# lms-org/trajectory_controller

Hardware: AMD Instinct MI355X
Metric: MPC QP solves/sec (horizon N=20, 2 inputs) at 1/2/4/8 MI355X; max|du| vs dlib (higher is better)
Workload: dtype f64; 1 GPU; batch 262144 trajectories per GPU, N=20, 2 inputs, compact (mpcControllerTobi) form, cold start, eps 0.01, max_iter 10000; global_batch=262144, horizon=20, algo=lane_fma, parallelism=batch-sharded x1, batches_in_flight=1, gather=none (1 GPU)

## Files before the change

trajectory_controller_amd/csrc/mpc_ub.h:

```cpp
#pragma once

#include "mpc_lane.h"
#include "mpc_ub_model.h"

namespace tpc {

template <typename T, bool EQB> TPC_DEV void ub_set_uniform(ub::Unit<T, EQB>& m, T gscale, const CompactArgs& g) {
    const T q[2] = {(T)g.q[0], (T)g.q[1]}, r[2] = {(T)g.r[0], (T)g.r[1]};
    const T lo[2] = {(T)g.lo[0], (T)g.lo[1]}, hi[2] = {(T)g.hi[0], (T)g.hi[1]};
    m.set_uniform(gscale, q, r, lo, hi);
}

template <typename T, int H> struct UbCdPlan {
    static constexpr bool mirror = 2 * (2 * H * kWave * (int)sizeof(T)) <= 64 * 1024 &&
                                   2 * (2 * H * kWave * (int)sizeof(T)) * 4 * CdOcc<T, H>::value <= 160 * 1024;
    static constexpr bool x_in_lds = mirror && sizeof(T) == 8 && H >= 20;
    static constexpr bool fast = true;
};

TPC_DEV double cd_ldexp(double x, int e) { return __builtin_ldexp(x, e); }
TPC_DEV float cd_ldexp(float x, int e) { return __builtin_ldexpf(x, e); }

template <typename T, int H, bool EQB>
__global__ __launch_bounds__(64, (CdOcc<T, H>::value)) void ub_cd_kernel(CompactArgs g, Knobs kn, T* __restrict__ recs,
                                                                         uint32_t* __restrict__ keys,
                                                                         uint32_t* __restrict__ key_rank,
                                                                         uint32_t* __restrict__ key_hist,
                                                                         unsigned long long* __restrict__ stats) {
    using P = UbCdPlan<T, H>;
    constexpr int RL = LaneRec<T, H>::kLen;
    constexpr bool MIRROR = P::mirror, XL = P::x_in_lds;
    __shared__ T s_iqd[2 * H][kWave];
    __shared__ T s_x[MIRROR ? 2 * H : 1][kWave];
    const int lane = threadIdx.x;
    const int64_t k = (int64_t)blockIdx.x * kWave + lane;
    if (k >= g.n) return;

    ub::Unit<T, EQB> m;
    ub_set_uniform(m, (T)1, g);
    const T ty = ((const T*)g.dy)[k], tphi = ((const T*)g.dphi)[k];
    m.set_instance((T)g.step, (T)g.wheelbase, ((const T*)g.v)[k], ty, tphi);
    const bool nonfinite = m.nonfinite_inputs(ty, tphi);
    const T q0 = (T)g.q[0], q1 = (T)g.q[1], r0 = (T)g.r[0], r1 = (T)g.r[1];

    T x[XL ? 1 : 2 * H], w[ub::Reverse<T, H>::value ? 1 : 2 * H];
    auto X = [&](int q) -> T { if constexpr (XL) return s_x[q][lane]; else return x[q]; };
#pragma unroll
    for (int q = 0; q < 2 * H; ++q) {
        if constexpr (!XL) x[q] = m.xz(q & 1);
        if constexpr (MIRROR) s_x[q][lane] = m.xz(q & 1);
    }
    const T lambda = ub::ctor_lambda_qdiag<T, H>(m.a, m.c, q0, q1, r0, r1, [&](int i, int j, T val) {
        s_iqd[2 * i + j][lane] = val != (T)0 ? (T)1 / (val * m.s(j)) : (T)0;
    });
    const T eps = (T)kn.eps;
    const bool screen_ok = ub::fast_stop_ok(m, ty, tphi, q0, q1, r0, r1, eps, lambda);
    const unsigned long long failing = __ballot(!screen_ok);
    if (failing != 0ull && lane == __ffsll((long long)failing) - 1) atomicOr(&stats[2], 1ull);
    if constexpr (sizeof(T) == 4) {
        const unsigned long long unmoved = __ballot(!ub::moved_stop_ok(m, eps, lambda));
        if (unmoved != 0ull && lane == __ffsll((long long)unmoved) - 1) atomicOr(&stats[2], 2ull);
    }
    const uint32_t cd_iters = kn.smo_iters < kn.max_iter ? kn.smo_iters : kn.max_iter;
    uint32_t iter = 0;
    bool stopped = nonfinite;
    bool vinit = false;
    constexpr T kHuge = (T)(sizeof(T) == 8 ? 0x1p600 : 0x1p100);
    T huge = kHuge;
    asm volatile("" : "+v"(huge));

    auto iteration = [&](auto fast_tag, uint32_t it) {
        constexpr bool F = decltype(fast_tag)::value;
        constexpr bool RV = ub::Reverse<T, H>::value;
        T Z, Y;
        m.fwd_init(Z, Y);
#pragma unroll
        for (int i = 0; i < H; ++i) {
            m.fwd(Z, Y, X(2 * i), X(2 * i + 1));
            if constexpr (!RV) { w[2 * i] = Z; w[2 * i + 1] = Y; }
        }
        T n0, n1;
        m.bwd_last(n0, n1, Z, Y);
        T max_df = (T)0, best_x = (T)0, best_mm = (T)0;
        int best = 0, best_sign = 0;
#pragma unroll
        for (int i = H - 1; i >= 0; --i) {
            if (i < H - 1) {
                if constexpr (RV) m.bwd(n0, n1, Z, Y); else m.bwd(n0, n1, w[2 * i], w[2 * i + 1]);
            }
            const T xi[2] = {X(2 * i), X(2 * i + 1)};
#pragma unroll
            for (int j = 1; j >= 0; --j) {
                const int q = 2 * i + j;
                const T xx = xi[j];
                const T dd = j == 0 ? m.df0(n1, xx) : m.df1(n0, n1, xx);
                if constexpr (F) {
                    T g_lo, g_hi;
                    if constexpr (ub::Unit<T, EQB>::kUnitBox) { g_lo = cd_ldexp(xx, 1900); g_hi = cd_ldexp((T)1 - xx, 1900); }
                    else { g_lo = m.gap_lo(j, xx, huge); g_hi = m.gap_hi(j, xx, huge); }
                    const T mm = tmax(tmin(dd, g_lo), -g_hi);
                    const bool better = tabs(mm) >= tabs(best_mm);
                    best_mm = better ? mm : best_mm;
                    best = better ? q : best;
                    if constexpr (!MIRROR) best_x = better ? xx : best_x;
                } else {
                    const T up = (xx <= m.bl(j)) ? (T)0 : dd;
                    const T dn = (xx >= m.bh(j)) ? (T)0 : -dd;
                    const T mag = tmax(up, dn);
                    const bool better = mag >= max_df && mag > (T)0;
                    max_df = tmax(max_df, mag);
                    best = better ? q : best;
                    best_sign = better ? sign_word(dd) : best_sign;
                    if constexpr (!MIRROR) best_x = better ? xx : best_x;
                }
            }
            if constexpr (RV) { if (i > 0) m.rev(Z, Y, xi[0], xi[1]); }
        }
        if constexpr (F) max_df = tabs(best_mm);
        stopped = stopped || max_df < eps;
        const bool act = !stopped;
        T best_df;
        if constexpr (F) best_df = best_mm; else best_df = with_sign(max_df, best_sign);
        if constexpr (MIRROR) best_x = s_x[best][lane];
        const T iq = s_iqd[best][lane];
        const bool upd = act && iq != (T)0;
        const T nx = m.project(ub::fma_(-iq, best_df, best_x), best & 1);
        if constexpr (MIRROR) { if (upd) s_x[best][lane] = nx; }
        if constexpr (!XL) {
            const int sel = upd ? best : -1;
#pragma unroll
            for (int q = 0; q < 2 * H; ++q) x[q] = (q == sel) ? nx : x[q];
        }
        vinit = upd ? (it + 1 == kn.smo_iters) : vinit;
        iter += act ? 1u : 0u;
    };
    if (P::fast && failing == 0ull) {
#pragma unroll 1
        for (uint32_t it = 0; it < cd_iters; ++it) {
            if (__ballot(!stopped) == 0ull) break;
            iteration(std::true_type{}, it);
        }
    } else {
#pragma unroll 1
        for (uint32_t it = 0; it < cd_iters; ++it) {
            if (__ballot(!stopped) == 0ull) break;
            iteration(std::false_type{}, it);
        }
    }

    T* rec = recs + (int64_t)k * RL;
#pragma unroll
    for (int q = 0; q < 2 * H; ++q) rec[q] = X(q);
    rec[2 * H] = lambda;
    uint64_t meta = (uint64_t)iter;
    if (stopped) meta |= kMetaStopped;
    if (vinit) meta |= kMetaVInit;
    if (nonfinite) meta |= kMetaNonFinite;
    store_meta<T>(rec + 2 * H + 1, meta);
    {
        T il0, il1, beta;
        ub::pg_constants<T>(lambda, m.s0, m.s1, il0, il1, beta);
        T* ex = rec + LaneRec<T, H>::kExtra;
        ex[0] = il0; ex[1] = il1; ex[2] = beta; ex[3] = m.a; ex[4] = m.c; ex[5] = ty; ex[6] = tphi;
    }
    const bool finished = stopped || iter >= kn.max_iter;
    const T lambda_floor = (r0 + r1) * (T)H;
    const bool uninformative = lambda < (T)1.5 * lambda_floor;
    const float lf = g.work_hint ? (float)(g.work_hint[k] > 0 ? g.work_hint[k] : 1) : (float)lambda;
    const uint32_t spread = (uint32_t)k & 127u;
    uint32_t key = __float_as_uint(lf);
    if (finished) key = spread << 16;
    else if (!g.work_hint && uninformative) key = (0x7f00u + spread) << 16;
    else if (!(lf > 0.0f) || key < 0x00800000u) key = 0x00800000u;
    else if (key >= 0x7f000000u) key = 0x7effffffu;
    uint32_t f = 0;
    if (finished) {
        ((T*)g.front)[k] = nonfinite ? (T)0 : m.control(0, X(0));
        ((T*)g.rear)[k] = nonfinite ? (T)0 : m.control(1, X(1));
        if (g.iters) g.iters[k] = (int32_t)iter;
        if (nonfinite) f |= 0x1u;
        if (!stopped) f |= 0x2u;
    }
    raise_flags(g.flags, f);
    keys[k] = key;
    key_rank[k] = atomicAdd(&key_hist[key >> 16], 1u);
}

#ifndef TPC_UB_OCC
#define TPC_UB_OCC 0
#endif
#ifndef TPC_UB_KV
#define TPC_UB_KV -1
#endif
template <typename T, int H> struct UbPlan {
    static constexpr bool D = sizeof(T) == 8;
    static constexpr int words = D ? 2 : 1;
    static constexpr bool reverse = ub::Reverse<T, H>::value;
    static constexpr bool regs = 6 * H * words <= 200 || !D || (reverse && 4 * H * words <= 200);
    static constexpr int occ_default = D ? 1 : ((H == 10 || H == 20) ? 2 : 1);
    static constexpr int occ = TPC_UB_OCC > 0 ? TPC_UB_OCC : occ_default;
    static constexpr int kv_default = regs ? H : (H == 20 ? 16 : (H == 30 ? 8 : 16));
    static constexpr int kv = regs ? H : (TPC_UB_KV >= 0 ? TPC_UB_KV : kv_default);
    static constexpr bool step_barrier = H - kv >= 8;
};
template <int H> struct UbRefillBatch { static constexpr int value = RefillBatch<H>::value; };

template <typename T, int H, bool EQB, int MODE>
__global__ __launch_bounds__((64 * UbPlan<T, H>::occ), (UbPlan<T, H>::occ)) void ub_pg_kernel(
    CompactArgs g, Knobs kn, const T* __restrict__ recs, const uint32_t* __restrict__ order,
    uint32_t* __restrict__ ticket, unsigned long long* __restrict__ stats, const uint32_t* __restrict__ queue_len) {
    using P = UbPlan<T, H>;
    constexpr int RL = LaneRec<T, H>::kLen;
    const int64_t n_queue = (int64_t)__builtin_nontemporal_load(queue_len);
    constexpr bool FAST = MODE != 0;
    static_assert(MODE == 0 || MODE == 2 || (MODE == 1 && sizeof(T) == 4), "the mask-as-arithmetic build is fp32's");
    {
        const unsigned long long sel = __builtin_nontemporal_load(&stats[2]);
        const int need = (sel & 1ull) ? 0 : ((sizeof(T) == 4 && (sel & 2ull)) ? 1 : 2);
        if (need != MODE) return;
        if (n_queue <= 0) return;
    }
    constexpr int BT = kWave * P::occ;
    constexpr int KV = P::kv, VL = H - KV;
// ... 213 lines not shown
```

Before: 58.23 million solves/s.

## Replace f64 coordinate-descent inner loop with hand-scheduled inline GCN assembly

For f64, H=20 with equality bounds and x in LDS, the fast coordinate-descent loop is replaced by a generated inline-asm loop. It batches LDS reads with explicit waitcnt interleaving, runs the forward and backward recurrences as FMA chains, does the argmax selection with cndmask, and writes the projected update back to LDS under an exec mask. The two shared arrays are merged into one contiguous buffer so fixed st64 offsets can address them. This is meant to cut compiler scheduling overhead and per-iteration branching. In exchange it hard-codes about 178 VGPRs, which may limit occupancy. It also uses a clamp-based projection and ldexp bounds tricks that must match the C++ semantics.

```diff
diff --git a/trajectory_controller_amd/csrc/mpc_ub.h b/trajectory_controller_amd/csrc/mpc_ub.h
--- a/trajectory_controller_amd/csrc/mpc_ub.h
+++ b/trajectory_controller_amd/csrc/mpc_ub.h
@@ -2,6 +2,7 @@
 
 #include "mpc_lane.h"
 #include "mpc_ub_model.h"
+#include "mpc_ub_cd_asm.h"
 
 namespace tpc {
 
@@ -16,6 +17,14 @@
                                    2 * (2 * H * kWave * (int)sizeof(T)) * 4 * CdOcc<T, H>::value <= 160 * 1024;
     static constexpr bool x_in_lds = mirror && sizeof(T) == 8 && H >= 20;
     static constexpr bool fast = true;
+};
+
+template <typename T, int H, bool EQB> struct UbCdAsm {
+#ifdef TPC_UB_CD_NO_ASM
+    static constexpr bool value = false;
+#else
+    static constexpr bool value = sizeof(T) == 8 && H == kUbCdAsmH && EQB && UbCdPlan<T, H>::x_in_lds;
+#endif
 };
 
 TPC_DEV double cd_ldexp(double x, int e) { return __builtin_ldexp(x, e); }
@@ -30,8 +39,9 @@
     using P = UbCdPlan<T, H>;
     constexpr int RL = LaneRec<T, H>::kLen;
     constexpr bool MIRROR = P::mirror, XL = P::x_in_lds;
-    __shared__ T s_iqd[2 * H][kWave];
-    __shared__ T s_x[MIRROR ? 2 * H : 1][kWave];
+    __shared__ T s_cd[2 * H + (MIRROR ? 2 * H : 1)][kWave];
+    T (*const s_iqd)[kWave] = s_cd;
+    T (*const s_x)[kWave] = s_cd + 2 * H;
     const int lane = threadIdx.x;
     const int64_t k = (int64_t)blockIdx.x * kWave + lane;
     if (k >= g.n) return;
@@ -135,10 +145,21 @@
         iter += act ? 1u : 0u;
     };
     if (P::fast && failing == 0ull) {
+        if constexpr (UbCdAsm<T, H, EQB>::value) {
+            static_assert(kUbCdAsmXRow == 2 * H, "LDS layout the generated loop reads");
+            const UbCdAsmUniform u = {m.gq0, m.gq1, m.grs0, m.grs1, m.lo1, (double)kn.eps};
+            uint64_t live = __ballot(!stopped);
+            uint32_t lu = 0;
+            const uint32_t vaddr = (uint32_t)(uintptr_t)&s_cd[0][lane];
+            ub_cd_asm_loop(u, m.a, m.c, m.as1, m.cs0, m.z0, m.q1th, m.grl0, m.grl1, vaddr, cd_iters, live, iter, lu);
+            stopped = ((live >> lane) & 1ull) == 0ull;
+            vinit = lu != 0u && lu == kn.smo_iters;
+        } else {
 #pragma unroll 1
-        for (uint32_t it = 0; it < cd_iters; ++it) {
-            if (__ballot(!stopped) == 0ull) break;
-            iteration(std::true_type{}, it);
+            for (uint32_t it = 0; it < cd_iters; ++it) {
+                if (__ballot(!stopped) == 0ull) break;
+                iteration(std::true_type{}, it);
+            }
         }
     } else {
 #pragma unroll 1
diff --git a/trajectory_controller_amd/csrc/mpc_ub_cd_asm.h b/trajectory_controller_amd/csrc/mpc_ub_cd_asm.h
--- /dev/null
+++ b/trajectory_controller_amd/csrc/mpc_ub_cd_asm.h
@@ -0,0 +1,667 @@
+#pragma once
+
+namespace tpc {
+
+constexpr int kUbCdAsmH = 20, kUbCdAsmIterInstrs = 627, kUbCdAsmXRow = 40;
+
+struct UbCdAsmUniform { double gq0, gq1, grs0, grs1, lo1, eps; };
+#pragma clang diagnostic push
+#pragma clang diagnostic ignored "-Winline-asm"
+TPC_DEV void ub_cd_asm_loop(const UbCdAsmUniform& u, double a, double c, double as1, double cs0, double z0, double q1th,
+                            double grl0, double grl1, uint32_t vaddr, uint32_t cd_iters, uint64_t& live,
+                            uint32_t& iter, uint32_t& lu) {
+    uint64_t sexec;
+    uint32_t sit;
+    asm volatile(
+        "s_waitcnt lgkmcnt(0)\n"
+        "s_mov_b64 %[sexec], exec\n"
+        "s_mov_b32 %[sit], 0\n"
+        ".p2align 3\n"
+        "TOP%=:\n"
+        "s_cmp_ge_u32 %[sit], %[scd]\n"
+        "s_cbranch_scc1 END%=\n"
+        "s_cmp_eq_u64 %[slive], 0\n"
+        "s_cbranch_scc1 END%=\n"
+        "ds_read2st64_b64 v[0:3], %[vaddr] offset0:40 offset1:41\n"
+        "ds_read2st64_b64 v[4:7], %[vaddr] offset0:42 offset1:43\n"
+        "ds_read2st64_b64 v[8:11], %[vaddr] offset0:44 offset1:45\n"
+        "ds_read2st64_b64 v[12:15], %[vaddr] offset0:46 offset1:47\n"
+        "ds_read2st64_b64 v[16:19], %[vaddr] offset0:48 offset1:49\n"
+        "ds_read2st64_b64 v[20:23], %[vaddr] offset0:50 offset1:51\n"
+        "ds_read2st64_b64 v[24:27], %[vaddr] offset0:52 offset1:53\n"
+        "ds_read2st64_b64 v[28:31], %[vaddr] offset0:54 offset1:55\n"
+        "ds_read2st64_b64 v[32:35], %[vaddr] offset0:56 offset1:57\n"
+        "ds_read2st64_b64 v[36:39], %[vaddr] offset0:58 offset1:59\n"
+        "ds_read2st64_b64 v[40:43], %[vaddr] offset0:60 offset1:61\n"
+        "ds_read2st64_b64 v[44:47], %[vaddr] offset0:62 offset1:63\n"
+        "ds_read2st64_b64 v[48:51], %[vaddr] offset0:64 offset1:65\n"
+        "ds_read2st64_b64 v[52:55], %[vaddr] offset0:66 offset1:67\n"
+        "ds_read2st64_b64 v[56:59], %[vaddr] offset0:68 offset1:69\n"
+        "s_waitcnt lgkmcnt(13)\n"
+        "s_nop 0\n"
+        "v_fma_f64 v[80:81], %[ca], %[slo1], %[cz0]\n"
+        "v_fma_f64 v[82:83], -%[ccs], v[2:3], %[slo1]\n"
+        "v_fma_f64 v[80:81], %[cas], v[2:3], v[80:81]\n"
+        "v_fma_f64 v[82:83], %[ccs], v[0:1], v[82:83]\n"
+        "ds_read2st64_b64 v[60:63], %[vaddr] offset0:70 offset1:71\n"
+        "v_fma_f64 v[84:85], %[ca], v[82:83], v[80:81]\n"
+        "v_fma_f64 v[86:87], -%[ccs], v[6:7], v[82:83]\n"
+        "v_fma_f64 v[84:85], %[cas], v[6:7], v[84:85]\n"
+        "v_fma_f64 v[86:87], %[ccs], v[4:5], v[86:87]\n"
+        "ds_read2st64_b64 v[64:67], %[vaddr] offset0:72 offset1:73\n"
+        "s_waitcnt lgkmcnt(13)\n"
+        "s_nop 0\n"
+        "v_fma_f64 v[88:89], %[ca], v[86:87], v[84:85]\n"
+        "v_fma_f64 v[90:91], -%[ccs], v[10:11], v[86:87]\n"
+        "v_fma_f64 v[88:89], %[cas], v[10:11], v[88:89]\n"
+        "v_fma_f64 v[90:91], %[ccs], v[8:9], v[90:91]\n"
+        "ds_read2st64_b64 v[68:71], %[vaddr] offset0:74 offset1:75\n"
+        "v_fma_f64 v[92:93], %[ca], v[90:91], v[88:89]\n"
+        "v_fma_f64 v[94:95], -%[ccs], v[14:15], v[90:91]\n"
+        "v_fma_f64 v[92:93], %[cas], v[14:15], v[92:93]\n"
+        "v_fma_f64 v[94:95], %[ccs], v[12:13], v[94:95]\n"
+        "ds_read2st64_b64 v[72:75], %[vaddr] offset0:76 offset1:77\n"
+        "s_waitcnt lgkmcnt(11)\n"
+        "s_nop 0\n"
+        "v_fma_f64 v[96:97], %[ca], v[94:95], v[92:93]\n"
+        "v_fma_f64 v[98:99], -%[ccs], v[18:19], v[94:95]\n"
+        "v_fma_f64 v[96:97], %[cas], v[18:19], v[96:97]\n"
+        "v_fma_f64 v[98:99], %[ccs], v[16:17], v[98:99]\n"
+        "ds_read2st64_b64 v[76:79], %[vaddr] offset0:78 offset1:79\n"
+        "v_fma_f64 v[100:101], %[ca], v[98:99], v[96:97]\n"
+        "v_fma_f64 v[102:103], -%[ccs], v[22:23], v[98:99]\n"
+        "v_fma_f64 v[100:101], %[cas], v[22:23], v[100:101]\n"
+        "v_fma_f64 v[102:103], %[ccs], v[20:21], v[102:103]\n"
+        "v_fma_f64 v[104:105], %[ca], v[102:103], v[100:101]\n"
+        "v_fma_f64 v[106:107], -%[ccs], v[26:27], v[102:103]\n"
+        "v_fma_f64 v[104:105], %[cas], v[26:27], v[104:105]\n"
+        "v_fma_f64 v[106:107], %[ccs], v[24:25], v[106:107]\n"
+        "v_fma_f64 v[108:109], %[ca], v[106:107], v[104:105]\n"
+        "v_fma_f64 v[110:111], -%[ccs], v[30:31], v[106:107]\n"
+        "v_fma_f64 v[108:109], %[cas], v[30:31], v[108:109]\n"
+        "v_fma_f64 v[110:111], %[ccs], v[28:29], v[110:111]\n"
+        "s_waitcnt lgkmcnt(8)\n"
+        "s_nop 0\n"
+        "v_fma_f64 v[112:113], %[ca], v[110:111], v[108:109]\n"
+        "v_fma_f64 v[114:115], -%[ccs], v[34:35], v[110:111]\n"
+        "v_fma_f64 v[112:113], %[cas], v[34:35], v[112:113]\n"
+        "v_fma_f64 v[114:115], %[ccs], v[32:33], v[114:115]\n"
+        "v_fma_f64 v[116:117], %[ca], v[114:115], v[112:113]\n"
+        "v_fma_f64 v[118:119], -%[ccs], v[38:39], v[114:115]\n"
+        "v_fma_f64 v[116:117], %[cas], v[38:39], v[116:117]\n"
+        "v_fma_f64 v[118:119], %[ccs], v[36:37], v[118:119]\n"
+        "v_fma_f64 v[120:121], %[ca], v[118:119], v[116:117]\n"
+        "v_fma_f64 v[122:123], -%[ccs], v[42:43], v[118:119]\n"
+        "v_fma_f64 v[120:121], %[cas], v[42:43], v[120:121]\n"
+        "v_fma_f64 v[122:123], %[ccs], v[40:41], v[122:123]\n"
+        "v_fma_f64 v[124:125], %[ca], v[122:123], v[120:121]\n"
+        "v_fma_f64 v[126:127], -%[ccs], v[46:47], v[122:123]\n"
+        "v_fma_f64 v[124:125], %[cas], v[46:47], v[124:125]\n"
+        "v_fma_f64 v[126:127], %[ccs], v[44:45], v[126:127]\n"
+        "s_waitcnt lgkmcnt(4)\n"
+        "s_nop 0\n"
+        "v_fma_f64 v[128:129], %[ca], v[126:127], v[124:125]\n"
+        "v_fma_f64 v[130:131], -%[ccs], v[50:51], v[126:127]\n"
+        "v_fma_f64 v[128:129], %[cas], v[50:51], v[128:129]\n"
+        "v_fma_f64 v[130:131], %[ccs], v[48:49], v[130:131]\n"
+        "v_fma_f64 v[132:133], %[ca], v[130:131], v[128:129]\n"
+        "v_fma_f64 v[134:135], -%[ccs], v[54:55], v[130:131]\n"
+        "v_fma_f64 v[132:133], %[cas], v[54:55], v[132:133]\n"
+        "v_fma_f64 v[134:135], %[ccs], v[52:53], v[134:135]\n"
+        "v_fma_f64 v[136:137], %[ca], v[134:135], v[132:133]\n"
+        "v_fma_f64 v[138:139], -%[ccs], v[58:59], v[134:135]\n"
+        "v_fma_f64 v[136:137], %[cas], v[58:59], v[136:137]\n"
+        "v_fma_f64 v[138:139], %[ccs], v[56:57], v[138:139]\n"
+        "v_fma_f64 v[140:141], %[ca], v[138:139], v[136:137]\n"
+        "v_fma_f64 v[142:143], -%[ccs], v[62:63], v[138:139]\n"
+        "v_fma_f64 v[140:141], %[cas], v[62:63], v[140:141]\n"
+        "v_fma_f64 v[142:143], %[ccs], v[60:61], v[142:143]\n"
+        "s_waitcnt lgkmcnt(0)\n"
+        "s_nop 0\n"
+        "v_fma_f64 v[144:145], %[ca], v[142:143], v[140:141]\n"
+        "v_fma_f64 v[146:147], -%[ccs], v[66:67], v[142:143]\n"
+        "v_fma_f64 v[144:145], %[cas], v[66:67], v[144:145]\n"
+        "v_fma_f64 v[146:147], %[ccs], v[64:65], v[146:147]\n"
+        "v_fma_f64 v[148:149], %[ca], v[146:147], v[144:145]\n"
+        "v_fma_f64 v[150:151], -%[ccs], v[70:71], v[146:147]\n"
+        "v_fma_f64 v[148:149], %[cas], v[70:71], v[148:149]\n"
+        "v_fma_f64 v[150:151], %[ccs], v[68:69], v[150:151]\n"
+        "v_fma_f64 v[152:153], %[ca], v[150:151], v[148:149]\n"
+        "v_fma_f64 v[154:155], -%[ccs], v[74:75], v[150:151]\n"
+        "v_fma_f64 v[152:153], %[cas], v[74:75], v[152:153]\n"
+        "v_fma_f64 v[154:155], %[ccs], v[72:73], v[154:155]\n"
+        "v_fma_f64 v[156:157], %[ca], v[154:155], v[152:153]\n"
+        "v_fma_f64 v[158:159], -%[ccs], v[78:79], v[154:155]\n"
+        "v_fma_f64 v[156:157], %[cas], v[78:79], v[156:157]\n"
+        "v_fma_f64 v[158:159], %[ccs], v[76:77], v[158:159]\n"
+        "v_mul_f64 v[160:161], %[sgq0], v[156:157]\n"
+        "v_fma_f64 v[162:163], %[sgq1], v[158:159], -%[cq]\n"
+        "v_fma_f64 v[164:165], %[sgrs1], v[78:79], %[cgl1]\n"
+        "v_fma_f64 v[164:165], -%[cc], v[162:163], v[164:165]\n"
+        "v_fma_f64 v[164:165], %[ca], v[160:161], v[164:165]\n"
+        "v_ldexp_f64 v[166:167], v[78:79], %[s1900]\n"
+        "v_fma_f64 v[168:169], -v[78:79], %[sbig], %[sbig]\n"
+        "v_min_f64 v[170:171], v[164:165], v[166:167]\n"
+        "v_max_f64 v[170:171], v[170:171], -v[168:169]\n"
+        "v_fma_f64 v[164:165], %[sgrs0], v[76:77], %[cgl0]\n"
+        "v_fma_f64 v[164:165], %[cc], v[162:163], v[164:165]\n"
+        "v_ldexp_f64 v[166:167], v[76:77], %[s1900]\n"
+        "v_fma_f64 v[168:169], -v[76:77], %[sbig], %[sbig]\n"
+        "v_min_f64 v[166:167], v[164:165], v[166:167]\n"
+        "v_max_f64 v[166:167], v[166:167], -v[168:169]\n"
+        "v_cmp_lt_f64_e64 vcc, |v[166:167]|, |v[170:171]|\n"
+        "v_cndmask_b32_e64 v170, v166, v170, vcc\n"
+        "v_cndmask_b32_e64 v171, v167, v171, vcc\n"
+        "v_cndmask_b32_e64 v172, 38, 39, vcc\n"
+        "v_fma_f64 v[154:155], %[sgq1], v[154:155], -%[cq]\n"
+        "v_fma_f64 v[162:163], %[ca], v[160:161], v[162:163]\n"
+        "v_add_f64 v[162:163], v[162:163], v[154:155]\n"
+        "v_fma_f64 v[160:161], %[sgq0], v[152:153], v[160:161]\n"
+        "v_fma_f64 v[164:165], %[sgrs1], v[74:75], %[cgl1]\n"
+        "v_fma_f64 v[164:165], -%[cc], v[162:163], v[164:165]\n"
+        "v_fma_f64 v[164:165], %[ca], v[160:161], v[164:165]\n"
+        "v_ldexp_f64 v[166:167], v[74:75], %[s1900]\n"
+        "v_fma_f64 v[168:169], -v[74:75], %[sbig], %[sbig]\n"
+        "v_min_f64 v[166:167], v[164:165], v[166:167]\n"
+        "v_max_f64 v[166:167], v[166:167], -v[168:169]\n"
+        "v_cmp_lt_f64_e64 vcc, |v[166:167]|, |v[170:171]|\n"
+        "v_cndmask_b32_e64 v170, v166, v170, vcc\n"
+        "v_cndmask_b32_e64 v171, v167, v171, vcc\n"
+        "v_cndmask_b32_e64 v172, 37, v172, vcc\n"
+        "v_fma_f64 v[164:165], %[sgrs0], v[72:73], %[cgl0]\n"
+        "v_fma_f64 v[164:165], %[cc], v[162:163], v[164:165]\n"
+        "v_ldexp_f64 v[166:167], v[72:73], %[s1900]\n"
+        "v_fma_f64 v[168:169], -v[72:73], %[sbig], %[sbig]\n"
+        "v_min_f64 v[166:167], v[164:165], v[166:167]\n"
+        "v_max_f64 v[166:167], v[166:167], -v[168:169]\n"
+        "v_cmp_lt_f64_e64 vcc, |v[166:167]|, |v[170:171]|\n"
+        "v_cndmask_b32_e64 v170, v166, v170, vcc\n"
+        "v_cndmask_b32_e64 v171, v167, v171, vcc\n"
+        "v_cndmask_b32_e64 v172, 36, v172, vcc\n"
+        "v_fma_f64 v[150:151], %[sgq1], v[150:151], -%[cq]\n"
+        "v_fma_f64 v[162:163], %[ca], v[160:161], v[162:163]\n"
+        "v_add_f64 v[162:163], v[162:163], v[150:151]\n"
+        "v_fma_f64 v[160:161], %[sgq0], v[148:149], v[160:161]\n"
+        "v_fma_f64 v[164:165], %[sgrs1], v[70:71], %[cgl1]\n"
+        "v_fma_f64 v[164:165], -%[cc], v[162:163], v[164:165]\n"
+        "v_fma_f64 v[164:165], %[ca], v[160:161], v[164:165]\n"
+        "v_ldexp_f64 v[166:167], v[70:71], %[s1900]\n"
+        "v_fma_f64 v[168:169], -v[70:71], %[sbig], %[sbig]\n"
+        "v_min_f64 v[166:167], v[164:165], v[166:167]\n"
+        "v_max_f64 v[166:167], v[166:167], -v[168:169]\n"
+        "v_cmp_lt_f64_e64 vcc, |v[166:167]|, |v[170:171]|\n"
+        "v_cndmask_b32_e64 v170, v166, v170, vcc\n"
+        "v_cndmask_b32_e64 v171, v167, v171, vcc\n"
+        "v_cndmask_b32_e64 v172, 35, v172, vcc\n"
+        "v_fma_f64 v[164:165], %[sgrs0], v[68:69], %[cgl0]\n"
+        "v_fma_f64 v[164:165], %[cc], v[162:163], v[164:165]\n"
+        "v_ldexp_f64 v[166:167], v[68:69], %[s1900]\n"
+        "v_fma_f64 v[168:169], -v[68:69], %[sbig], %[sbig]\n"
+        "v_min_f64 v[166:167], v[164:165], v[166:167]\n"
+        "v_max_f64 v[166:167], v[166:167], -v[168:169]\n"
+        "v_cmp_lt_f64_e64 vcc, |v[166:167]|, |v[170:171]|\n"
+        "v_cndmask_b32_e64 v170, v166, v170, vcc\n"
+        "v_cndmask_b32_e64 v171, v167, v171, vcc\n"
+        "v_cndmask_b32_e64 v172, 34, v172, vcc\n"
+        "v_fma_f64 v[146:147], %[sgq1], v[146:147], -%[cq]\n"
+        "v_fma_f64 v[162:163], %[ca], v[160:161], v[162:163]\n"
+        "v_add_f64 v[162:163], v[162:163], v[146:147]\n"
+        "v_fma_f64 v[160:161], %[sgq0], v[144:145], v[160:161]\n"
+        "v_fma_f64 v[164:165], %[sgrs1], v[66:67], %[cgl1]\n"
+        "v_fma_f64 v[164:165], -%[cc], v[162:163], v[164:165]\n"
+        "v_fma_f64 v[164:165], %[ca], v[160:161], v[164:165]\n"
+        "v_ldexp_f64 v[166:167], v[66:67], %[s1900]\n"
+        "v_fma_f64 v[168:169], -v[66:67], %[sbig], %[sbig]\n"
+        "v_min_f64 v[166:167], v[164:165], v[166:167]\n"
+        "v_max_f64 v[166:167], v[166:167], -v[168:169]\n"
+        "v_cmp_lt_f64_e64 vcc, |v[166:167]|, |v[170:171]|\n"
+        "v_cndmask_b32_e64 v170, v166, v170, vcc\n"
+        "v_cndmask_b32_e64 v171, v167, v171, vcc\n"
+        "v_cndmask_b32_e64 v172, 33, v172, vcc\n"
+        "v_fma_f64 v[164:165], %[sgrs0], v[64:65], %[cgl0]\n"
+        "v_fma_f64 v[164:165], %[cc], v[162:163], v[164:165]\n"
+        "v_ldexp_f64 v[166:167], v[64:65], %[s1900]\n"
+        "v_fma_f64 v[168:169], -v[64:65], %[sbig], %[sbig]\n"
+        "v_min_f64 v[166:167], v[164:165], v[166:167]\n"
+        "v_max_f64 v[166:167], v[166:167], -v[168:169]\n"
+        "v_cmp_lt_f64_e64 vcc, |v[166:167]|, |v[170:171]|\n"
+        "v_cndmask_b32_e64 v170, v166, v170, vcc\n"
+        "v_cndmask_b32_e64 v171, v167, v171, vcc\n"
+        "v_cndmask_b32_e64 v172, 32, v172, vcc\n"
+        "v_fma_f64 v[142:143], %[sgq1], v[142:143], -%[cq]\n"
+        "v_fma_f64 v[162:163], %[ca], v[160:161], v[162:163]\n"
+        "v_add_f64 v[162:163], v[162:163], v[142:143]\n"
+        "v_fma_f64 v[160:161], %[sgq0], v[140:141], v[160:161]\n"
+        "v_fma_f64 v[164:165], %[sgrs1], v[62:63], %[cgl1]\n"
+        "v_fma_f64 v[164:165], -%[cc], v[162:163], v[164:165]\n"
+        "v_fma_f64 v[164:165], %[ca], v[160:161], v[164:165]\n"
+        "v_ldexp_f64 v[166:167], v[62:63], %[s1900]\n"
+        "v_fma_f64 v[168:169], -v[62:63], %[sbig], %[sbig]\n"
+        "v_min_f64 v[166:167], v[164:165], v[166:167]\n"
+        "v_max_f64 v[166:167], v[166:167], -v[168:169]\n"
+        "v_cmp_lt_f64_e64 vcc, |v[166:167]|, |v[170:171]|\n"
+        "v_cndmask_b32_e64 v170, v166, v170, vcc\n"
+        "v_cndmask_b32_e64 v171, v167, v171, vcc\n"
+        "v_cndmask_b32_e64 v172, 31, v172, vcc\n"
+        "v_fma_f64 v[164:165], %[sgrs0], v[60:61], %[cgl0]\n"
+        "v_fma_f64 v[164:165], %[cc], v[162:163], v[164:165]\n"
+        "v_ldexp_f64 v[166:167], v[60:61], %[s1900]\n"
+        "v_fma_f64 v[168:169], -v[60:61], %[sbig], %[sbig]\n"
+        "v_min_f64 v[166:167], v[164:165], v[166:167]\n"
+        "v_max_f64 v[166:167], v[166:167], -v[168:169]\n"
+        "v_cmp_lt_f64_e64 vcc, |v[166:167]|, |v[170:171]|\n"
+        "v_cndmask_b32_e64 v170, v166, v170, vcc\n"
+        "v_cndmask_b32_e64 v171, v167, v171, vcc\n"
+        "v_cndmask_b32_e64 v172, 30, v172, vcc\n"
+        "v_fma_f64 v[138:139], %[sgq1], v[138:139], -%[cq]\n"
+        "v_fma_f64 v[162:163], %[ca], v[160:161], v[162:163]\n"
+        "v_add_f64 v[162:163], v[162:163], v[138:139]\n"
+        "v_fma_f64 v[160:161], %[sgq0], v[136:137], v[160:161]\n"
+        "v_fma_f64 v[164:165], %[sgrs1], v[58:59], %[cgl1]\n"
+        "v_fma_f64 v[164:165], -%[cc], v[162:163], v[164:165]\n"
+        "v_fma_f64 v[164:165], %[ca], v[160:161], v[164:165]\n"
+        "v_ldexp_f64 v[166:167], v[58:59], %[s1900]\n"
+        "v_fma_f64 v[168:169], -v[58:59], %[sbig], %[sbig]\n"
+        "v_min_f64 v[166:167], v[164:165], v[166:167]\n"
+        "v_max_f64 v[166:167], v[166:167], -v[168:169]\n"
+        "v_cmp_lt_f64_e64 vcc, |v[166:167]|, |v[170:171]|\n"
+        "v_cndmask_b32_e64 v170, v166, v170, vcc\n"
+        "v_cndmask_b32_e64 v171, v167, v171, vcc\n"
+        "v_cndmask_b32_e64 v172, 29, v172, vcc\n"
+        "v_fma_f64 v[164:165], %[sgrs0], v[56:57], %[cgl0]\n"
+        "v_fma_f64 v[164:165], %[cc], v[162:163], v[164:165]\n"
+        "v_ldexp_f64 v[166:167], v[56:57], %[s1900]\n"
+        "v_fma_f64 v[168:169], -v[56:57], %[sbig], %[sbig]\n"
+        "v_min_f64 v[166:167], v[164:165], v[166:167]\n"
+        "v_max_f64 v[166:167], v[166:167], -v[168:169]\n"
+        "v_cmp_lt_f64_e64 vcc, |v[166:167]|, |v[170:171]|\n"
+        "v_cndmask_b32_e64 v170, v166, v170, vcc\n"
+        "v_cndmask_b32_e64 v171, v167, v171, vcc\n"
+        "v_cndmask_b32_e64 v172, 28, v172, vcc\n"
+        "v_fma_f64 v[134:135], %[sgq1], v[134:135], -%[cq]\n"
+        "v_fma_f64 v[162:163], %[ca], v[160:161], v[162:163]\n"
+        "v_add_f64 v[162:163], v[162:163], v[134:135]\n"
+        "v_fma_f64 v[160:161], %[sgq0], v[132:133], v[160:161]\n"
+        "v_fma_f64 v[164:165], %[sgrs1], v[54:55], %[cgl1]\n"
+        "v_fma_f64 v[164:165], -%[cc], v[162:163], v[164:165]\n"
+        "v_fma_f64 v[164:165], %[ca], v[160:161], v[164:165]\n"
+        "v_ldexp_f64 v[166:167], v[54:55], %[s1900]\n"
+        "v_fma_f64 v[168:169], -v[54:55], %[sbig], %[sbig]\n"
+        "v_min_f64 v[166:167], v[164:165], v[166:167]\n"
+        "v_max_f64 v[166:167], v[166:167], -v[168:169]\n"
+        "v_cmp_lt_f64_e64 vcc, |v[166:167]|, |v[170:171]|\n"
+        "v_cndmask_b32_e64 v170, v166, v170, vcc\n"
+        "v_cndmask_b32_e64 v171, v167, v171, vcc\n"
+        "v_cndmask_b32_e64 v172, 27, v172, vcc\n"
+        "v_fma_f64 v[164:165], %[sgrs0], v[52:53], %[cgl0]\n"
+        "v_fma_f64 v[164:165], %[cc], v[162:163], v[164:165]\n"
+        "v_ldexp_f64 v[166:167], v[52:53], %[s1900]\n"
+        "v_fma_f64 v[168:169], -v[52:53], %[sbig], %[sbig]\n"
+        "v_min_f64 v[166:167], v[164:165], v[166:167]\n"
+        "v_max_f64 v[166:167], v[166:167], -v[168:169]\n"
+        "v_cmp_lt_f64_e64 vcc, |v[166:167]|, |v[170:171]|\n"
+        "v_cndmask_b32_e64 v170, v166, v170, vcc\n"
+        "v_cndmask_b32_e64 v171, v167, v171, vcc\n"
+        "v_cndmask_b32_e64 v172, 26, v172, vcc\n"
+        "v_fma_f64 v[130:131], %[sgq1], v[130:131], -%[cq]\n"
+        "v_fma_f64 v[162:163], %[ca], v[160:161], v[162:163]\n"
+        "v_add_f64 v[162:163], v[162:163], v[130:131]\n"
+        "v_fma_f64 v[160:161], %[sgq0], v[128:129], v[160:161]\n"
+        "v_fma_f64 v[164:165], %[sgrs1], v[50:51], %[cgl1]\n"
+        "v_fma_f64 v[164:165], -%[cc], v[162:163], v[164:165]\n"
+        "v_fma_f64 v[164:165], %[ca], v[160:161], v[164:165]\n"
+        "v_ldexp_f64 v[166:167], v[50:51], %[s1900]\n"
+        "v_fma_f64 v[168:169], -v[50:51], %[sbig], %[sbig]\n"
+        "v_min_f64 v[166:167], v[164:165], v[166:167]\n"
+        "v_max_f64 v[166:167], v[166:167], -v[168:169]\n"
+        "v_cmp_lt_f64_e64 vcc, |v[166:167]|, |v[170:171]|\n"
+        "v_cndmask_b32_e64 v170, v166, v170, vcc\n"
+        "v_cndmask_b32_e64 v171, v167, v171, vcc\n"
+        "v_cndmask_b32_e64 v172, 25, v172, vcc\n"
+        "v_fma_f64 v[164:165], %[sgrs0], v[48:49], %[cgl0]\n"
+        "v_fma_f64 v[164:165], %[cc], v[162:163], v[164:165]\n"
+        "v_ldexp_f64 v[166:167], v[48:49], %[s1900]\n"
+        "v_fma_f64 v[168:169], -v[48:49], %[sbig], %[sbig]\n"
+        "v_min_f64 v[166:167], v[164:165], v[166:167]\n"
+        "v_max_f64 v[166:167], v[166:167], -v[168:169]\n"
+        "v_cmp_lt_f64_e64 vcc, |v[166:167]|, |v[170:171]|\n"
+        "v_cndmask_b32_e64 v170, v166, v170, vcc\n"
+        "v_cndmask_b32_e64 v171, v167, v171, vcc\n"
+        "v_cndmask_b32_e64 v172, 24, v172, vcc\n"
+        "v_fma_f64 v[126:127], %[sgq1], v[126:127], -%[cq]\n"
+        "v_fma_f64 v[162:163], %[ca], v[160:161], v[162:163]\n"
+        "v_add_f64 v[162:163], v[162:163], v[126:127]\n"
+        "v_fma_f64 v[160:161], %[sgq0], v[124:125], v[160:161]\n"
+        "v_fma_f64 v[164:165], %[sgrs1], v[46:47], %[cgl1]\n"
+        "v_fma_f64 v[164:165], -%[cc], v[162:163], v[164:165]\n"
+        "v_fma_f64 v[164:165], %[ca], v[160:161], v[164:165]\n"
+        "v_ldexp_f64 v[166:167], v[46:47], %[s1900]\n"
+        "v_fma_f64 v[168:169], -v[46:47], %[sbig], %[sbig]\n"
+        "v_min_f64 v[166:167], v[164:165], v[166:167]\n"
+        "v_max_f64 v[166:167], v[166:167], -v[168:169]\n"
+        "v_cmp_lt_f64_e64 vcc, |v[166:167]|, |v[170:171]|\n"
+        "v_cndmask_b32_e64 v170, v166, v170, vcc\n"
+        "v_cndmask_b32_e64 v171, v167, v171, vcc\n"
+        "v_cndmask_b32_e64 v172, 23, v172, vcc\n"
+        "v_fma_f64 v[164:165], %[sgrs0], v[44:45], %[cgl0]\n"
+        "v_fma_f64 v[164:165], %[cc], v[162:163], v[164:165]\n"
+        "v_ldexp_f64 v[166:167], v[44:45], %[s1900]\n"
+        "v_fma_f64 v[168:169], -v[44:45], %[sbig], %[sbig]\n"
+        "v_min_f64 v[166:167], v[164:165], v[166:167]\n"
+        "v_max_f64 v[166:167], v[166:167], -v[168:169]\n"
+        "v_cmp_lt_f64_e64 vcc, |v[166:167]|, |v[170:171]|\n"
+        "v_cndmask_b32_e64 v170, v166, v170, vcc\n"
+        "v_cndmask_b32_e64 v171, v167, v171, vcc\n"
+        "v_cndmask_b32_e64 v172, 22, v172, vcc\n"
+        "v_fma_f64 v[122:123], %[sgq1], v[122:123], -%[cq]\n"
+        "v_fma_f64 v[162:163], %[ca], v[160:161], v[162:163]\n"
+        "v_add_f64 v[162:163], v[162:163], v[122:123]\n"
+        "v_fma_f64 v[160:161], %[sgq0], v[120:121], v[160:161]\n"
+        "v_fma_f64 v[164:165], %[sgrs1], v[42:43], %[cgl1]\n"
+        "v_fma_f64 v[164:165], -%[cc], v[162:163], v[164:165]\n"
+        "v_fma_f64 v[164:165], %[ca], v[160:161], v[164:165]\n"
+        "v_ldexp_f64 v[166:167], v[42:43], %[s1900]\n"
+        "v_fma_f64 v[168:169], -v[42:43], %[sbig], %[sbig]\n"
+        "v_min_f64 v[166:167], v[164:165], v[166:167]\n"
+        "v_max_f64 v[166:167], v[166:167], -v[168:169]\n"
+        "v_cmp_lt_f64_e64 vcc, |v[166:167]|, |v[170:171]|\n"
+        "v_cndmask_b32_e64 v170, v166, v170, vcc\n"
+        "v_cndmask_b32_e64 v171, v167, v171, vcc\n"
+        "v_cndmask_b32_e64 v172, 21, v172, vcc\n"
+        "v_fma_f64 v[164:165], %[sgrs0], v[40:41], %[cgl0]\n"
+        "v_fma_f64 v[164:165], %[cc], v[162:163], v[164:165]\n"
+        "v_ldexp_f64 v[166:167], v[40:41], %[s1900]\n"
+        "v_fma_f64 v[168:169], -v[40:41], %[sbig], %[sbig]\n"
+        "v_min_f64 v[166:167], v[164:165], v[166:167]\n"
+        "v_max_f64 v[166:167], v[166:167], -v[168:169]\n"
+        "v_cmp_lt_f64_e64 vcc, |v[166:167]|, |v[170:171]|\n"
+        "v_cndmask_b32_e64 v170, v166, v170, vcc\n"
+        "v_cndmask_b32_e64 v171, v167, v171, vcc\n"
+        "v_cndmask_b32_e64 v172, 20, v172, vcc\n"
+        "v_fma_f64 v[118:119], %[sgq1], v[118:119], -%[cq]\n"
+        "v_fma_f64 v[162:163], %[ca], v[160:161], v[162:163]\n"
+        "v_add_f64 v[162:163], v[162:163], v[118:119]\n"
+        "v_fma_f64 v[160:161], %[sgq0], v[116:117], v[160:161]\n"
+        "v_fma_f64 v[164:165], %[sgrs1], v[38:39], %[cgl1]\n"
+        "v_fma_f64 v[164:165], -%[cc], v[162:163], v[164:165]\n"
+        "v_fma_f64 v[164:165], %[ca], v[160:161], v[164:165]\n"
+        "v_ldexp_f64 v[166:167], v[38:39], %[s1900]\n"
+        "v_fma_f64 v[168:169], -v[38:39], %[sbig], %[sbig]\n"
+        "v_min_f64 v[166:167], v[164:165], v[166:167]\n"
+        "v_max_f64 v[166:167], v[166:167], -v[168:169]\n"
+        "v_cmp_lt_f64_e64 vcc, |v[166:167]|, |v[170:171]|\n"
+        "v_cndmask_b32_e64 v170, v166, v170, vcc\n"
+        "v_cndmask_b32_e64 v171, v167, v171, vcc\n"
+        "v_cndmask_b32_e64 v172, 19, v172, vcc\n"
+        "v_fma_f64 v[164:165], %[sgrs0], v[36:37], %[cgl0]\n"
+        "v_fma_f64 v[164:165], %[cc], v[162:163], v[164:165]\n"
+        "v_ldexp_f64 v[166:167], v[36:37], %[s1900]\n"
+        "v_fma_f64 v[168:169], -v[36:37], %[sbig], %[sbig]\n"
+        "v_min_f64 v[166:167], v[164:165], v[166:167]\n"
+        "v_max_f64 v[166:167], v[166:167], -v[168:169]\n"
+        "v_cmp_lt_f64_e64 vcc, |v[166:167]|, |v[170:171]|\n"
+        "v_cndmask_b32_e64 v170, v166, v170, vcc\n"
+        "v_cndmask_b32_e64 v171, v167, v171, vcc\n"
+        "v_cndmask_b32_e64 v172, 18, v172, vcc\n"
+        "v_fma_f64 v[114:115], %[sgq1], v[114:115], -%[cq]\n"
+        "v_fma_f64 v[162:163], %[ca], v[160:161], v[162:163]\n"
+        "v_add_f64 v[162:163], v[162:163], v[114:115]\n"
+        "v_fma_f64 v[160:161], %[sgq0], v[112:113], v[160:161]\n"
+        "v_fma_f64 v[164:165], %[sgrs1], v[34:35], %[cgl1]\n"
+        "v_fma_f64 v[164:165], -%[cc], v[162:163], v[164:165]\n"
+        "v_fma_f64 v[164:165], %[ca], v[160:161], v[164:165]\n"
+        "v_ldexp_f64 v[166:167], v[34:35], %[s1900]\n"
+        "v_fma_f64 v[168:169], -v[34:35], %[sbig], %[sbig]\n"
+        "v_min_f64 v[166:167], v[164:165], v[166:167]\n"
+        "v_max_f64 v[166:167], v[166:167], -v[168:169]\n"
+        "v_cmp_lt_f64_e64 vcc, |v[166:167]|, |v[170:171]|\n"
+        "v_cndmask_b32_e64 v170, v166, v170, vcc\n"
+        "v_cndmask_b32_e64 v171, v167, v171, vcc\n"
+        "v_cndmask_b32_e64 v172, 17, v172, vcc\n"
+        "v_fma_f64 v[164:165], %[sgrs0], v[32:33], %[cgl0]\n"
+        "v_fma_f64 v[164:165], %[cc], v[162:163], v[164:165]\n"
+        "v_ldexp_f64 v[166:167], v[32:33], %[s1900]\n"
+        "v_fma_f64 v[168:169], -v[32:33], %[sbig], %[sbig]\n"
+        "v_min_f64 v[166:167], v[164:165], v[166:167]\n"
+        "v_max_f64 v[166:167], v[166:167], -v[168:169]\n"
+        "v_cmp_lt_f64_e64 vcc, |v[166:167]|, |v[170:171]|\n"
+        "v_cndmask_b32_e64 v170, v166, v170, vcc\n"
+        "v_cndmask_b32_e64 v171, v167, v171, vcc\n"
+        "v_cndmask_b32_e64 v172, 16, v172, vcc\n"
+        "v_fma_f64 v[110:111], %[sgq1], v[110:111], -%[cq]\n"
+        "v_fma_f64 v[162:163], %[ca], v[160:161], v[162:163]\n"
+        "v_add_f64 v[162:163], v[162:163], v[110:111]\n"
+        "v_fma_f64 v[160:161], %[sgq0], v[108:109], v[160:161]\n"
+        "v_fma_f64 v[164:165], %[sgrs1], v[30:31], %[cgl1]\n"
+        "v_fma_f64 v[164:165], -%[cc], v[162:163], v[164:165]\n"
+        "v_fma_f64 v[164:165], %[ca], v[160:161], v[164:165]\n"
+        "v_ldexp_f64 v[166:167], v[30:31], %[s1900]\n"
+        "v_fma_f64 v[168:169], -v[30:31], %[sbig], %[sbig]\n"
+        "v_min_f64 v[166:167], v[164:165], v[166:167]\n"
+        "v_max_f64 v[166:167], v[166:167], -v[168:169]\n"
+        "v_cmp_lt_f64_e64 vcc, |v[166:167]|, |v[170:171]|\n"
+        "v_cndmask_b32_e64 v170, v166, v170, vcc\n"
+        "v_cndmask_b32_e64 v171, v167, v171, vcc\n"
+        "v_cndmask_b32_e64 v172, 15, v172, vcc\n"
+        "v_fma_f64 v[164:165], %[sgrs0], v[28:29], %[cgl0]\n"
+        "v_fma_f64 v[164:165], %[cc], v[162:163], v[164:165]\n"
+        "v_ldexp_f64 v[166:167], v[28:29], %[s1900]\n"
+        "v_fma_f64 v[168:169], -v[28:29], %[sbig], %[sbig]\n"
+        "v_min_f64 v[166:167], v[164:165], v[166:167]\n"
+        "v_max_f64 v[166:167], v[166:167], -v[168:169]\n"
+        "v_cmp_lt_f64_e64 vcc, |v[166:167]|, |v[170:171]|\n"
+        "v_cndmask_b32_e64 v170, v166, v170, vcc\n"
+        "v_cndmask_b32_e64 v171, v167, v171, vcc\n"
+        "v_cndmask_b32_e64 v172, 14, v172, vcc\n"
+        "v_fma_f64 v[106:107], %[sgq1], v[106:107], -%[cq]\n"
+        "v_fma_f64 v[162:163], %[ca], v[160:161], v[162:163]\n"
+        "v_add_f64 v[162:163], v[162:163], v[106:107]\n"
+        "v_fma_f64 v[160:161], %[sgq0], v[104:105], v[160:161]\n"
+        "v_fma_f64 v[164:165], %[sgrs1], v[26:27], %[cgl1]\n"
+        "v_fma_f64 v[164:165], -%[cc], v[162:163], v[164:165]\n"
+        "v_fma_f64 v[164:165], %[ca], v[160:161], v[164:165]\n"
+        "v_ldexp_f64 v[166:167], v[26:27], %[s1900]\n"
+        "v_fma_f64 v[168:169], -v[26:27], %[sbig], %[sbig]\n"
+        "v_min_f64 v[166:167], v[164:165], v[166:167]\n"
+        "v_max_f64 v[166:167], v[166:167], -v[168:169]\n"
+        "v_cmp_lt_f64_e64 vcc, |v[166:167]|, |v[170:171]|\n"
+        "v_cndmask_b32_e64 v170, v166, v170, vcc\n"
+        "v_cndmask_b32_e64 v171, v167, v171, vcc\n"
+        "v_cndmask_b32_e64 v172, 13, v172, vcc\n"
+        "v_fma_f64 v[164:165], %[sgrs0], v[24:25], %[cgl0]\n"
+        "v_fma_f64 v[164:165], %[cc], v[162:163], v[164:165]\n"
+        "v_ldexp_f64 v[166:167], v[24:25], %[s1900]\n"
+        "v_fma_f64 v[168:169], -v[24:25], %[sbig], %[sbig]\n"
+        "v_min_f64 v[166:167], v[164:165], v[166:167]\n"
+        "v_max_f64 v[166:167], v[166:167], -v[168:169]\n"
+        "v_cmp_lt_f64_e64 vcc, |v[166:167]|, |v[170:171]|\n"
+        "v_cndmask_b32_e64 v170, v166, v170, vcc\n"
+        "v_cndmask_b32_e64 v171, v167, v171, vcc\n"
+        "v_cndmask_b32_e64 v172, 12, v172, vcc\n"
+        "v_fma_f64 v[102:103], %[sgq1], v[102:103], -%[cq]\n"
+        "v_fma_f64 v[162:163], %[ca], v[160:161], v[162:163]\n"
+        "v_add_f64 v[162:163], v[162:163], v[102:103]\n"
+        "v_fma_f64 v[160:161], %[sgq0], v[100:101], v[160:161]\n"
+        "v_fma_f64 v[164:165], %[sgrs1], v[22:23], %[cgl1]\n"
+        "v_fma_f64 v[164:165], -%[cc], v[162:163], v[164:165]\n"
+        "v_fma_f64 v[164:165], %[ca], v[160:161], v[164:165]\n"
+        "v_ldexp_f64 v[166:167], v[22:23], %[s1900]\n"
+        "v_fma_f64 v[168:169], -v[22:23], %[sbig], %[sbig]\n"
+        "v_min_f64 v[166:167], v[164:165], v[166:167]\n"
+        "v_max_f64 v[166:167], v[166:167], -v[168:169]\n"
+        "v_cmp_lt_f64_e64 vcc, |v[166:167]|, |v[170:171]|\n"
+        "v_cndmask_b32_e64 v170, v166, v170, vcc\n"
+        "v_cndmask_b32_e64 v171, v167, v171, vcc\n"
+        "v_cndmask_b32_e64 v172, 11, v172, vcc\n"
+        "v_fma_f64 v[164:165], %[sgrs0], v[20:21], %[cgl0]\n"
+        "v_fma_f64 v[164:165], %[cc], v[162:163], v[164:165]\n"
+        "v_ldexp_f64 v[166:167], v[20:21], %[s1900]\n"
+        "v_fma_f64 v[168:169], -v[20:21], %[sbig], %[sbig]\n"
+        "v_min_f64 v[166:167], v[164:165], v[166:167]\n"
+        "v_max_f64 v[166:167], v[166:167], -v[168:169]\n"
+        "v_cmp_lt_f64_e64 vcc, |v[166:167]|, |v[170:171]|\n"
+        "v_cndmask_b32_e64 v170, v166, v170, vcc\n"
+        "v_cndmask_b32_e64 v171, v167, v171, vcc\n"
+        "v_cndmask_b32_e64 v172, 10, v172, vcc\n"
+        "v_fma_f64 v[98:99], %[sgq1], v[98:99], -%[cq]\n"
+        "v_fma_f64 v[162:163], %[ca], v[160:161], v[162:163]\n"
+        "v_add_f64 v[162:163], v[162:163], v[98:99]\n"
+        "v_fma_f64 v[160:161], %[sgq0], v[96:97], v[160:161]\n"
+        "v_fma_f64 v[164:165], %[sgrs1], v[18:19], %[cgl1]\n"
+        "v_fma_f64 v[164:165], -%[cc], v[162:163], v[164:165]\n"
+        "v_fma_f64 v[164:165], %[ca], v[160:161], v[164:165]\n"
+        "v_ldexp_f64 v[166:167], v[18:19], %[s1900]\n"
+        "v_fma_f64 v[168:169], -v[18:19], %[sbig], %[sbig]\n"
+        "v_min_f64 v[166:167], v[164:165], v[166:167]\n"
+        "v_max_f64 v[166:167], v[166:167], -v[168:169]\n"
+        "v_cmp_lt_f64_e64 vcc, |v[166:167]|, |v[170:171]|\n"
+        "v_cndmask_b32_e64 v170, v166, v170, vcc\n"
+        "v_cndmask_b32_e64 v171, v167, v171, vcc\n"
+        "v_cndmask_b32_e64 v172, 9, v172, vcc\n"
+        "v_fma_f64 v[164:165], %[sgrs0], v[16:17], %[cgl0]\n"
+        "v_fma_f64 v[164:165], %[cc], v[162:163], v[164:165]\n"
+        "v_ldexp_f64 v[166:167], v[16:17], %[s1900]\n"
+        "v_fma_f64 v[168:169], -v[16:17], %[sbig], %[sbig]\n"
+        "v_min_f64 v[166:167], v[164:165], v[166:167]\n"
+        "v_max_f64 v[166:167], v[166:167], -v[168:169]\n"
+        "v_cmp_lt_f64_e64 vcc, |v[166:167]|, |v[170:171]|\n"
+        "v_cndmask_b32_e64 v170, v166, v170, vcc\n"
+        "v_cndmask_b32_e64 v171, v167, v171, vcc\n"
+        "v_cndmask_b32_e64 v172, 8, v172, vcc\n"
+        "v_fma_f64 v[94:95], %[sgq1], v[94:95], -%[cq]\n"
+        "v_fma_f64 v[162:163], %[ca], v[160:161], v[162:163]\n"
+        "v_add_f64 v[162:163], v[162:163], v[94:95]\n"
+        "v_fma_f64 v[160:161], %[sgq0], v[92:93], v[160:161]\n"
+        "v_fma_f64 v[164:165], %[sgrs1], v[14:15], %[cgl1]\n"
+        "v_fma_f64 v[164:165], -%[cc], v[162:163], v[164:165]\n"
+        "v_fma_f64 v[164:165], %[ca], v[160:161], v[164:165]\n"
+        "v_ldexp_f64 v[166:167], v[14:15], %[s1900]\n"
+        "v_fma_f64 v[168:169], -v[14:15], %[sbig], %[sbig]\n"
+        "v_min_f64 v[166:167], v[164:165], v[166:167]\n"
+        "v_max_f64 v[166:167], v[166:167], -v[168:169]\n"
+        "v_cmp_lt_f64_e64 vcc, |v[166:167]|, |v[170:171]|\n"
+        "v_cndmask_b32_e64 v170, v166, v170, vcc\n"
+        "v_cndmask_b32_e64 v171, v167, v171, vcc\n"
+        "v_cndmask_b32_e64 v172, 7, v172, vcc\n"
+        "v_fma_f64 v[164:165], %[sgrs0], v[12:13], %[cgl0]\n"
+        "v_fma_f64 v[164:165], %[cc], v[162:163], v[164:165]\n"
+        "v_ldexp_f64 v[166:167], v[12:13], %[s1900]\n"
+        "v_fma_f64 v[168:169], -v[12:13], %[sbig], %[sbig]\n"
+        "v_min_f64 v[166:167], v[164:165], v[166:167]\n"
+        "v_max_f64 v[166:167], v[166:167], -v[168:169]\n"
+        "v_cmp_lt_f64_e64 vcc, |v[166:167]|, |v[170:171]|\n"
+        "v_cndmask_b32_e64 v170, v166, v170, vcc\n"
+        "v_cndmask_b32_e64 v171, v167, v171, vcc\n"
+        "v_cndmask_b32_e64 v172, 6, v172, vcc\n"
+        "v_fma_f64 v[90:91], %[sgq1], v[90:91], -%[cq]\n"
+        "v_fma_f64 v[162:163], %[ca], v[160:161], v[162:163]\n"
+        "v_add_f64 v[162:163], v[162:163], v[90:91]\n"
+        "v_fma_f64 v[160:161], %[sgq0], v[88:89], v[160:161]\n"
+        "v_fma_f64 v[164:165], %[sgrs1], v[10:11], %[cgl1]\n"
+        "v_fma_f64 v[164:165], -%[cc], v[162:163], v[164:165]\n"
+        "v_fma_f64 v[164:165], %[ca], v[160:161], v[164:165]\n"
+        "v_ldexp_f64 v[166:167], v[10:11], %[s1900]\n"
+        "v_fma_f64 v[168:169], -v[10:11], %[sbig], %[sbig]\n"
+        "v_min_f64 v[166:167], v[164:165], v[166:167]\n"
+        "v_max_f64 v[166:167], v[166:167], -v[168:169]\n"
+        "v_cmp_lt_f64_e64 vcc, |v[166:167]|, |v[170:171]|\n"
+        "v_cndmask_b32_e64 v170, v166, v170, vcc\n"
+        "v_cndmask_b32_e64 v171, v167, v171, vcc\n"
+        "v_cndmask_b32_e64 v172, 5, v172, vcc\n"
+        "v_fma_f64 v[164:165], %[sgrs0], v[8:9], %[cgl0]\n"
+        "v_fma_f64 v[164:165], %[cc], v[162:163], v[164:165]\n"
+        "v_ldexp_f64 v[166:167], v[8:9], %[s1900]\n"
+        "v_fma_f64 v[168:169], -v[8:9], %[sbig], %[sbig]\n"
+        "v_min_f64 v[166:167], v[164:165], v[166:167]\n"
+        "v_max_f64 v[166:167], v[166:167], -v[168:169]\n"
+        "v_cmp_lt_f64_e64 vcc, |v[166:167]|, |v[170:171]|\n"
+        "v_cndmask_b32_e64 v170, v166, v170, vcc\n"
+        "v_cndmask_b32_e64 v171, v167, v171, vcc\n"
+        "v_cndmask_b32_e64 v172, 4, v172, vcc\n"
+        "v_fma_f64 v[86:87], %[sgq1], v[86:87], -%[cq]\n"
+        "v_fma_f64 v[162:163], %[ca], v[160:161], v[162:163]\n"
+        "v_add_f64 v[162:163], v[162:163], v[86:87]\n"
+        "v_fma_f64 v[160:161], %[sgq0], v[84:85], v[160:161]\n"
+        "v_fma_f64 v[164:165], %[sgrs1], v[6:7], %[cgl1]\n"
+        "v_fma_f64 v[164:165], -%[cc], v[162:163], v[164:165]\n"
+        "v_fma_f64 v[164:165], %[ca], v[160:161], v[164:165]\n"
+        "v_ldexp_f64 v[166:167], v[6:7], %[s1900]\n"
+        "v_fma_f64 v[168:169], -v[6:7], %[sbig], %[sbig]\n"
+        "v_min_f64 v[166:167], v[164:165], v[166:167]\n"
+        "v_max_f64 v[166:167], v[166:167], -v[168:169]\n"
+        "v_cmp_lt_f64_e64 vcc, |v[166:167]|, |v[170:171]|\n"
+        "v_cndmask_b32_e64 v170, v166, v170, vcc\n"
+        "v_cndmask_b32_e64 v171, v167, v171, vcc\n"
+        "v_cndmask_b32_e64 v172, 3, v172, vcc\n"
+        "v_fma_f64 v[164:165], %[sgrs0], v[4:5], %[cgl0]\n"
+        "v_fma_f64 v[164:165], %[cc], v[162:163], v[164:165]\n"
+        "v_ldexp_f64 v[166:167], v[4:5], %[s1900]\n"
+        "v_fma_f64 v[168:169], -v[4:5], %[sbig], %[sbig]\n"
+        "v_min_f64 v[166:167], v[164:165], v[166:167]\n"
+        "v_max_f64 v[166:167], v[166:167], -v[168:169]\n"
+        "v_cmp_lt_f64_e64 vcc, |v[166:167]|, |v[170:171]|\n"
+        "v_cndmask_b32_e64 v170, v166, v170, vcc\n"
+        "v_cndmask_b32_e64 v171, v167, v171, vcc\n"
+        "v_cndmask_b32_e64 v172, 2, v172, vcc\n"
+        "v_fma_f64 v[82:83], %[sgq1], v[82:83], -%[cq]\n"
+        "v_fma_f64 v[162:163], %[ca], v[160:161], v[162:163]\n"
+        "v_add_f64 v[162:163], v[162:163], v[82:83]\n"
+        "v_fma_f64 v[160:161], %[sgq0], v[80:81], v[160:161]\n"
+        "v_fma_f64 v[164:165], %[sgrs1], v[2:3], %[cgl1]\n"
+        "v_fma_f64 v[164:165], -%[cc], v[162:163], v[164:165]\n"
+        "v_fma_f64 v[164:165], %[ca], v[160:161], v[164:165]\n"
+        "v_ldexp_f64 v[166:167], v[2:3], %[s1900]\n"
+        "v_fma_f64 v[168:169], -v[2:3], %[sbig], %[sbig]\n"
+        "v_min_f64 v[166:167], v[164:165], v[166:167]\n"
+        "v_max_f64 v[166:167], v[166:167], -v[168:169]\n"
+        "v_cmp_lt_f64_e64 vcc, |v[166:167]|, |v[170:171]|\n"
+        "v_cndmask_b32_e64 v170, v166, v170, vcc\n"
+        "v_cndmask_b32_e64 v171, v167, v171, vcc\n"
+        "v_cndmask_b32_e64 v172, 1, v172, vcc\n"
+        "v_fma_f64 v[164:165], %[sgrs0], v[0:1], %[cgl0]\n"
+        "v_fma_f64 v[164:165], %[cc], v[162:163], v[164:165]\n"
+        "v_ldexp_f64 v[166:167], v[0:1], %[s1900]\n"
+        "v_fma_f64 v[168:169], -v[0:1], %[sbig], %[sbig]\n"
+        "v_min_f64 v[166:167], v[164:165], v[166:167]\n"
+        "v_max_f64 v[166:167], v[166:167], -v[168:169]\n"
+        "v_cmp_lt_f64_e64 vcc, |v[166:167]|, |v[170:171]|\n"
+        "v_cndmask_b32_e64 v170, v166, v170, vcc\n"
+        "v_cndmask_b32_e64 v171, v167, v171, vcc\n"
+        "v_cndmask_b32_e64 v172, 0, v172, vcc\n"
+        "v_lshl_add_u32 v173, v172, 9, %[vaddr]\n"
+        "ds_read2st64_b64 v[174:177], v173 offset0:40 offset1:0\n"
+        "v_cmp_lt_f64_e64 vcc, |v[170:171]|, %[seps]\n"
+        "s_andn2_b64 %[slive], %[slive], vcc\n"
+        "s_mov_b64 exec, %[slive]\n"
+        "v_add_u32_e64 %[viter], %[viter], 1\n"
+        "s_waitcnt lgkmcnt(0)\n"
+        "s_nop 0\n"
+        "v_cmp_neq_f64_e64 vcc, 0, v[176:177]\n"
+        "s_and_b64 exec, %[slive], vcc\n"
+        "s_nop 0\n"
+        "v_fma_f64 v[174:175], -v[176:177], v[170:171], v[174:175] clamp\n"
+        "v_add_u32_e64 %[vlu], %[sit], 1\n"
+        "ds_write_b64 v173, v[174:175] offset:20480\n"
+        "s_mov_b64 exec, %[sexec]\n"
+        "s_add_u32 %[sit], %[sit], 1\n"
+        "s_branch TOP%=\n"
+        "END%=:\n"
+        "s_mov_b64 exec, %[sexec]\n"
+        : [slive] "+s"(live), [viter] "+v"(iter), [vlu] "+v"(lu), [sexec] "=&s"(sexec), [sit] "=&s"(sit)
+        : [sgq0] "s"(u.gq0), [sgq1] "s"(u.gq1), [sgrs0] "s"(u.grs0), [sgrs1] "s"(u.grs1), [slo1] "s"(u.lo1), [seps] "s"(u.eps), [sbig] "s"(0x1p1000),
+          [s1900] "s"(1900), [scd] "s"(cd_iters), [ca] "v"(a), [cc] "v"(c), [cas] "v"(as1), [ccs] "v"(cs0), [cz0] "v"(z0), [cq] "v"(q1th), [cgl0] "v"(grl0),
+          [cgl1] "v"(grl1), [vaddr] "v"(vaddr)
+        : "v0", "v1", "v2", "v3", "v4", "v5", "v6", "v7", "v8", "v9", "v10", "v11", "v12", "v13", "v14", "v15", "v16", "v17", "v18", "v19", "v20", "v21",
+          "v22", "v23", "v24", "v25", "v26", "v27", "v28", "v29", "v30", "v31", "v32", "v33", "v34", "v35", "v36", "v37", "v38", "v39", "v40", "v41", "v42",
+          "v43", "v44", "v45", "v46", "v47", "v48", "v49", "v50", "v51", "v52", "v53", "v54", "v55", "v56", "v57", "v58", "v59", "v60", "v61", "v62", "v63",
+          "v64", "v65", "v66", "v67", "v68", "v69", "v70", "v71", "v72", "v73", "v74", "v75", "v76", "v77", "v78", "v79", "v80", "v81", "v82", "v83", "v84",
+          "v85", "v86", "v87", "v88", "v89", "v90", "v91", "v92", "v93", "v94", "v95", "v96", "v97", "v98", "v99", "v100", "v101", "v102", "v103", "v104",
+          "v105", "v106", "v107", "v108", "v109", "v110", "v111", "v112", "v113", "v114", "v115", "v116", "v117", "v118", "v119", "v120", "v121", "v122",
+          "v123", "v124", "v125", "v126", "v127", "v128", "v129", "v130", "v131", "v132", "v133", "v134", "v135", "v136", "v137", "v138", "v139", "v140",
+          "v141", "v142", "v143", "v144", "v145", "v146", "v147", "v148", "v149", "v150", "v151", "v152", "v153", "v154", "v155", "v156", "v157", "v158",
+          "v159", "v160", "v161", "v162", "v163", "v164", "v165", "v166", "v167", "v168", "v169", "v170", "v171", "v172", "v173", "v174", "v175", "v176",
+          "v177", "vcc", "scc", "exec", "memory");
+}
+#pragma clang diagnostic pop
+
+}
```

New measurement: 59.24 million solves/s (median of 6 runs). +1.7%, better.
